# robot-learning-freiburg/MM-DistillNet

Measured on AMD Instinct MI355X. Metric: distillation-step images/sec (3 teachers + audio student, D2, bs=8), higher is better.
Workload: dtype f32; 1 GPU; BASELINE configs[2]: full 3-teacher (RGB+thermal+depth) -> audio student distillation step, EfficientDet-D2, 512x512, per-GPU batch 8, fwd+losses+bwd+all-reduce+Adam; global_batch=8, image_size=512, parallelism=dp1, graph=True, full=False

## Files before the change

### mm_distillnet_amd/csrc/pw_rows.hip

```cpp
#include "common.h"
#include "pw_args.h"
#include <cstdlib>

#define RW_AFF 1
#define RW_SWISH 2
#define RW_GATE 4
#define RW_ABL_NOSTORE 256
#define RW_ABL_NOFETCH 512
#define RW_ABL_NOMFMA 1024

struct RowsArgs {
  int LDB;
  int nslabs;
  int spw;
  int cpp;
  int pcols;
  int npanels, bpp;
  int mode;
  int nlev;
};

typedef float f32x2 __attribute__((ext_vector_type(2)));
typedef __attribute__((address_space(3))) void* lds_vptr;
typedef const __attribute__((address_space(1))) void* glb_vptr;

template <int NKK, int C>
__global__ __launch_bounds__(512, 2) void pw_rows_kernel(PwArgs a, RowsArgs ra) {
  extern __shared__ float smem[];
  const int K = NKK * 8, N = a.N, LDB = ra.LDB, pcols = ra.pcols;
  float* const sB = smem;
  float* const sCoef = sB + pcols * LDB;
  float* const sEp = sCoef + 2 * K;
  float* const sStat = sEp + 3 * pcols;
  const int tid = threadIdx.x, lane = tid & 63, r = lane & 15, g = lane >> 4;
  const int wave = __builtin_amdgcn_readfirstlane(tid >> 6);
  const int panel = blockIdx.x / ra.bpp, bi = blockIdx.x - panel * ra.bpp;
  const int n0p = panel * pcols;

  const int slot = bi * 4 + (wave & 3), nslot = ra.bpp * 4;
  const int q_beg = (int)((long long)slot * ra.nslabs / nslot), q_end = (int)((long long)(slot + 1) * ra.nslabs / nslot);
  const int q_mid = q_beg + (q_end - q_beg + 1) / 2;
  const int s_beg = (wave < 4) ? q_beg : q_mid, s_end = (wave < 4) ? q_mid : q_end;
  f32x2 an[NKK], gn[NKK];
  int lev_n = 0, Mv_n = a.M, srow0_n = 0, rpi_n = a.rows_per_image;
    auto fetch = [&](int s) {
      const int row0 = s * 16;
      lev_n = 0; Mv_n = a.M; srow0_n = 0; rpi_n = a.rows_per_image;
      if (a.pyr.n) {
        lev_n = __builtin_amdgcn_readfirstlane(pyr_level_of_row(a.pyr, row0));
        srow0_n = a.pyr.row0[lev_n]; rpi_n = a.pyr.H[lev_n] * a.pyr.W[lev_n]; Mv_n = srow0_n + a.pyr.B * rpi_n;
      }
      const int row = min(row0 + r, Mv_n - 1);
      const float* xp = a.x + (size_t)row * K + 2 * g;
#pragma unroll
      for (int kk = 0; kk < NKK; ++kk) an[kk] = *reinterpret_cast<const f32x2*>(xp + kk * 8);
      if (ra.mode & RW_GATE) {
        const float* gp = a.gate + (size_t)(row / rpi_n) * K + 2 * g;
#pragma unroll
        for (int kk = 0; kk < NKK; ++kk) gn[kk] = *reinterpret_cast<const f32x2*>(gp + kk * 8);
      }
    };
  if (s_beg < s_end) fetch(s_beg);
  {
    const int f4 = K >> 2, spr = f4 + 1, total = pcols * spr;
    const int nI = (total + 63) >> 6;
    for (int ii = wave; ii < nI; ii += 8) {
      const int slot = ii * 64 + lane;
      const int n = slot / spr, k4 = slot - n * spr;
      const float* src = a.w + (size_t)min(n0p + n, N - 1) * K + min(k4, f4 - 1) * 4;
      if (slot < total && k4 < f4)
        __builtin_amdgcn_global_load_lds((glb_vptr)(uintptr_t)src, (lds_vptr)(uintptr_t)(sB + ii * 256), 16, 0, 0);
    }
    if (ra.mode & RW_AFF)
      for (int k = tid; k < K; k += 512) {
        float sc, sh;
        if (a.in_bn.stats) bn_live_coef(a.in_bn, k, sc, sh);
        else { sc = a.in_scale[k]; sh = a.in_shift[k]; }
        sCoef[k] = sc; sCoef[K + k] = sh;
      }
    for (int c = tid; c < pcols; c += 512) {
      const int col = n0p + c;
      const bool ok = col < N;
      sEp[c] = (a.bias && ok) ? a.bias[col] : 0.f;
      sEp[pcols + c] = (a.out_scale && ok) ? a.out_scale[col] : 1.f;
      sEp[2 * pcols + c] = (a.out_scale && ok) ? a.out_shift[col] : 0.f;
    }
    for (int i = tid; i < ra.nlev * 2 * pcols; i += 512) sStat[i] = 0.f;
  }
  asm volatile("s_waitcnt vmcnt(0)" ::: "memory");
  __syncthreads();

  if (s_beg < s_end) {
    for (int s = s_beg; s < s_end; ++s) {
      const int row0 = s * 16;
      const int lev = lev_n, Mv = Mv_n, srow0 = srow0_n, rpi = rpi_n;
      f32x2 ac[NKK];
#pragma unroll
      for (int kk = 0; kk < NKK; ++kk) ac[kk] = an[kk];
      if (ra.mode & RW_AFF) {
#pragma unroll
        for (int kk = 0; kk < NKK; ++kk) {
          const f32x2 sc = *reinterpret_cast<const f32x2*>(&sCoef[kk * 8 + 2 * g]);
          const f32x2 sh = *reinterpret_cast<const f32x2*>(&sCoef[K + kk * 8 + 2 * g]);
          ac[kk].x = ac[kk].x * sc.x + sh.x; ac[kk].y = ac[kk].y * sc.y + sh.y;
        }
      }
      if (ra.mode & RW_SWISH) {
#pragma unroll
        for (int kk = 0; kk < NKK; ++kk) { ac[kk].x = mmd_swish(ac[kk].x); ac[kk].y = mmd_swish(ac[kk].y); }
      }
      if (ra.mode & RW_GATE) {
#pragma unroll
        for (int kk = 0; kk < NKK; ++kk) { ac[kk].x *= gn[kk].x; ac[kk].y *= gn[kk].y; }
      }
      if (s + 1 < s_end && !(ra.mode & RW_ABL_NOFETCH)) fetch(s + 1);
      const bool rows_full = row0 + 16 <= Mv;
      size_t off[4]; bool rok[4];
#pragma unroll
      for (int i = 0; i < 4; ++i) {
        const int row = row0 + 4 * g + i;
        rok[i] = row < Mv;
        const int rr = rok[i] ? row : row0;
        if (a.y_batch_stride) {
          const int img = (rr - srow0) / rpi;
          const long long yoff = a.pyr.n ? a.yoff_lev[lev] : a.y_offset;
          off[i] = (size_t)img * a.y_batch_stride + yoff + (size_t)(rr - srow0 - img * rpi) * N;
        } else {
          off[i] = (size_t)rr * N;
        }
      }
      for (int ch = 0; ch < ra.cpp; ++ch) {
        const int cbase = ch * C * 16;
        if (n0p + cbase >= N) break;
        const bool full = rows_full && (n0p + cbase + C * 16 <= N);
        const int c0 = n0p + cbase + r;
        float res[C][4];
        if (a.residual) {
#pragma unroll
          for (int j = 0; j < C; ++j)
#pragma unroll
            for (int i = 0; i < 4; ++i) res[j][i] = (c0 + j * 16 < N && rok[i]) ? a.residual[off[i] + c0 + j * 16] : 0.f;
        }
        f32x4 acc[C];
#pragma unroll
        for (int j = 0; j < C; ++j) acc[j] = f32x4{0.f, 0.f, 0.f, 0.f};
        typedef const __attribute__((address_space(3))) f32x2* lds_f2p;
        const unsigned bp0 = (unsigned)(uintptr_t)(lds_vptr)(uintptr_t)(sB + (cbase + r) * LDB + 2 * g);
#pragma unroll
        for (int kk = 0; kk < NKK; ++kk) {
          if ((ra.mode & RW_ABL_NOMFMA) && kk > 0) break;
          f32x2 b[C];
          unsigned bpk = bp0 + kk * 32;
          asm volatile("" : "+v"(bpk));
#pragma unroll
          for (int j = 0; j < C; ++j) b[j] = *(lds_f2p)(uintptr_t)(bpk + j * 16 * LDB * 4);
#pragma unroll
          for (int j = 0; j < C; ++j) acc[j] = __builtin_amdgcn_mfma_f32_16x16x4f32(ac[kk].x, b[j].x, acc[j], 0, 0, 0);
#pragma unroll
          for (int j = 0; j < C; ++j) acc[j] = __builtin_amdgcn_mfma_f32_16x16x4f32(ac[kk].y, b[j].y, acc[j], 0, 0, 0);
        }
        const float* ep = sEp + cbase + r;
        if (a.bias) {
#pragma unroll
          for (int j = 0; j < C; ++j) { const float bias = ep[j * 16]; acc[j] += bias; }
        }
        if (ra.nlev) {
#pragma unroll
          for (int j = 0; j < C; ++j) {
            float ssum = 0.f, ssq = 0.f;
            const bool cok = c0 + j * 16 < N;
#pragma unroll
            for (int i = 0; i < 4; ++i) {
              const float v = (full || (cok && rok[i])) ? acc[j][i] : 0.f;
              ssum += v; ssq += v * v;
            }
            ssum += __shfl_xor(ssum, 16, 64); ssq += __shfl_xor(ssq, 16, 64);
            ssum += __shfl_xor(ssum, 32, 64); ssq += __shfl_xor(ssq, 32, 64);
            if (g == 0 && cok) {
              atomicAdd(&sStat[(lev * 2) * pcols + cbase + j * 16 + r], ssum);
              atomicAdd(&sStat[(lev * 2 + 1) * pcols + cbase + j * 16 + r], ssq);
            }
          }
        }
        if (a.out_scale) {
#pragma unroll
          for (int j = 0; j < C; ++j) { const float osc = ep[pcols + j * 16], osh = ep[2 * pcols + j * 16]; acc[j] = acc[j] * osc + osh; }
        }
        if (a.out_act == MMD_ACT_SWISH) {
#pragma unroll
          for (int j = 0; j < C; ++j)
#pragma unroll
            for (int i = 0; i < 4; ++i) acc[j][i] = mmd_swish(acc[j][i]);
        } else if (a.out_act == MMD_ACT_SIGMOID) {
#pragma unroll
          for (int j = 0; j < C; ++j)
#pragma unroll
            for (int i = 0; i < 4; ++i) acc[j][i] = mmd_sigmoid(acc[j][i]);
        }
        if (a.residual) {
#pragma unroll
          for (int j = 0; j < C; ++j)
#pragma unroll
            for (int i = 0; i < 4; ++i) acc[j][i] += res[j][i];
        }
        if (!(ra.mode & RW_ABL_NOSTORE)) {
          float* yp[4];
#pragma unroll
          for (int i = 0; i < 4; ++i) yp[i] = a.y + off[i] + c0;
          if (full) {
#pragma unroll
            for (int j = 0; j < C; ++j)
#pragma unroll
              for (int i = 0; i < 4; ++i) yp[i][j * 16] = acc[j][i];
          } else {
#pragma unroll
            for (int j = 0; j < C; ++j)
#pragma unroll
              for (int i = 0; i < 4; ++i)
                if (c0 + j * 16 < N && rok[i]) yp[i][j * 16] = acc[j][i];
          }
        }
      }
    }
  }
  if (ra.nlev) {
    __syncthreads();
    double* base = a.stats_ws ? a.stats_ws + (size_t)(blockIdx.x % a.ws_slots) * 2 * N : a.stats;
    for (int i = tid; i < ra.nlev * 2 * pcols; i += 512) {
      const int l = i / (2 * pcols), rem = i - l * 2 * pcols, which = rem / pcols, c = rem - which * pcols;
      const int col = n0p + c;
      const float v = sStat[i];
      if (col < N && v != 0.f) atomicAdd(&base[(a.pyr.n ? 2 * (size_t)l * a.lev_stride : 0) + (size_t)which * N + col], (double)v);
    }
  }
}

typedef void (*RowsKern)(PwArgs, RowsArgs);
template <int C>
static RowsKern rows_pick_k(int nkk) {
  switch (nkk) {
    case 2: return pw_rows_kernel<2, C>;
    case 3: return pw_rows_kernel<3, C>;
    case 4: return pw_rows_kernel<4, C>;
    case 6: return pw_rows_kernel<6, C>;
    case 11: return pw_rows_kernel<11, C>;
    case 12: return pw_rows_kernel<12, C>;
    case 14: return pw_rows_kernel<14, C>;
    case 15: return pw_rows_kernel<15, C>;
    case 16: return pw_rows_kernel<16, C>;
    default: return nullptr;
  }
}
static RowsKern rows_pick(int nkk, int c) {
  return c == 7 ? rows_pick_k<7>(nkk) : c == 4 ? rows_pick_k<4>(nkk) : c == 3 ? rows_pick_k<3>(nkk) : c == 1 ? rows_pick_k<1>(nkk) : nullptr;
}


int pw_rows_try(PwArgs& a, hipStream_t stream) {
  static const int off = getenv("MMD_NO_ROWS") ? 1 : 0;
  static const int lds_blk = getenv("MMD_ROWS_LDS") ? atoi(getenv("MMD_ROWS_LDS")) : 120 * 1024;
  if (off || a.bf16 || a.bb.z || a.xs.z || a.st.Cin) return 0;
  const int M = a.M, K = a.K, N = a.N;
  if (K < 16 || K > 128 || (K & 7)) return 0;
  static const int all = getenv("MMD_ROWS_ALL") ? 1 : 0;
  if (a.form == MMD_PW_FORM_TILED || a.form == MMD_PW_FORM_LONGK || a.form == MMD_PW_FORM_SLAB) return 0;
  if (!all && a.form != MMD_PW_FORM_ROWS && (M < 32768 || a.stats || N < 48)) return 0;
  if (a.in_act != MMD_ACT_NONE && a.in_act != MMD_ACT_SWISH) return 0;
  if (a.gate && (a.pyr.n || (a.rows_per_image & 15))) return 0;
  const int nkk = K / 8;
  const int tiles = cdiv(N, 16);
  const int nslabs = cdiv(M, 16);
  int C = 1; double best = -1.0;
  const int cands[4] = {7, 4, 3, 1};
  for (int ci = 0; ci < 4; ++ci) {
    const int c = cands[ci];
    const double eff = (double)tiles / (cdiv(tiles, c) * c) * (c == 1 ? 0.85 : 1.0);
    if (eff > best + 1e-9) { best = eff; C = c; }
  }
  static const int small_slabs = getenv("MMD_ROWS_SMALL") ? atoi(getenv("MMD_ROWS_SMALL")) : 512;
  if (nslabs * cdiv(tiles, C) < small_slabs && nslabs < small_slabs) C = 1;
  RowsKern kern = rows_pick(nkk, C);
  if (!kern) return 0;
  RowsArgs ra{};
  ra.LDB = K + 4;
  ra.nslabs = nslabs;
  const int nchunks = cdiv(tiles, C);
  const int chunk_bytes = C * 16 * ra.LDB * 4;
  int cpp = lds_blk / chunk_bytes; if (cpp < 1) cpp = 1; if (cpp > nchunks) cpp = nchunks;
  while (cpp > 1 && (long long)nslabs * cdiv(nchunks, cpp) < 1024) --cpp;
  ra.cpp = cpp; ra.pcols = cpp * C * 16; ra.npanels = cdiv(nchunks, cpp);
  ra.mode = ((a.in_scale || a.in_bn.stats) ? RW_AFF : 0) | (a.in_act == MMD_ACT_SWISH ? RW_SWISH : 0) | (a.gate ? RW_GATE : 0);
  static const int abl = (getenv("MMD_DEV") && getenv("MMD_ROWS_ABL")) ? atoi(getenv("MMD_ROWS_ABL")) : 0;
  ra.mode |= abl;
  ra.nlev = a.stats ? (a.pyr.n ? a.pyr.n : 1) : 0;
  const size_t lds = ((size_t)ra.pcols * ra.LDB + 2 * K + 3 * ra.pcols + (size_t)ra.nlev * 2 * ra.pcols) * sizeof(float);
  if (lds > 150 * 1024) return 0;
  static const int blk_target = getenv("MMD_ROWS_BLK") ? atoi(getenv("MMD_ROWS_BLK")) : 256;
  int maxblk = blk_target;
  if (a.stats && !a.stats_ws && maxblk > 128 * ra.npanels) maxblk = 128 * ra.npanels;
  int bpp = maxblk / ra.npanels; if (bpp < 1) bpp = 1;
  if (bpp > cdiv(nslabs, 8)) bpp = cdiv(nslabs, 8);
  ra.spw = cdiv(nslabs, bpp * 4);
  ra.bpp = bpp;
  static bool attr_done[17][8];
  if (!attr_done[nkk][C]) {
    hipFuncSetAttribute((const void*)kern, hipFuncAttributeMaxDynamicSharedMemorySize, 160 * 1024);
    attr_done[nkk][C] = true;
  }
  hipLaunchKernelGGL(kern, dim3(ra.npanels * bpp), dim3(512), lds, stream, a, ra);
  return 1;
}
```

Baseline: 602.7 images/sec.

## Fuse BN-backward prologue and preceding BN/swish grad reductions into rows pointwise kernel

Adds a BB template variant of the rows pointwise kernel that evaluates the batch-norm/activation backward on the input operand in the prologue. It optionally writes dz, accumulates dgamma/dbeta, and fuses per-image reductions for a following swish/BN backward (p5) into the epilogue through LDS and atomics. Previously these backward pointwise GEMMs fell back to other kernel forms, with separate elementwise and reduction passes. The change adds LDS use, atomics and restrictive eligibility conditions, and uses a larger block count for small-LDS cases.

```diff
diff --git a/mm_distillnet_amd/csrc/pw_rows.hip b/mm_distillnet_amd/csrc/pw_rows.hip
--- a/mm_distillnet_amd/csrc/pw_rows.hip
+++ b/mm_distillnet_amd/csrc/pw_rows.hip
@@ -24,14 +24,17 @@
 typedef __attribute__((address_space(3))) void* lds_vptr;
 typedef const __attribute__((address_space(1))) void* glb_vptr;
 
-template <int NKK, int C>
+template <int NKK, int C, int BB = 0>
 __global__ __launch_bounds__(512, 2) void pw_rows_kernel(PwArgs a, RowsArgs ra) {
   extern __shared__ float smem[];
   const int K = NKK * 8, N = a.N, LDB = ra.LDB, pcols = ra.pcols;
+  constexpr int NCO = BB ? 5 : 2;
   float* const sB = smem;
   float* const sCoef = sB + pcols * LDB;
-  float* const sEp = sCoef + 2 * K;
+  float* const sEp = sCoef + NCO * K;
   float* const sStat = sEp + 3 * pcols;
+  float* const sP5c = sStat + ra.nlev * 2 * pcols;
+  float* const sP5 = sP5c + 4 * pcols;
   const int tid = threadIdx.x, lane = tid & 63, r = lane & 15, g = lane >> 4;
   const int wave = __builtin_amdgcn_readfirstlane(tid >> 6);
   const int panel = blockIdx.x / ra.bpp, bi = blockIdx.x - panel * ra.bpp;
@@ -42,6 +45,7 @@
   const int q_mid = q_beg + (q_end - q_beg + 1) / 2;
   const int s_beg = (wave < 4) ? q_beg : q_mid, s_end = (wave < 4) ? q_mid : q_end;
   f32x2 an[NKK], gn[NKK];
+  float rs_n = 1.f;
   int lev_n = 0, Mv_n = a.M, srow0_n = 0, rpi_n = a.rows_per_image;
     auto fetch = [&](int s) {
       const int row0 = s * 16;
@@ -54,7 +58,12 @@
       const float* xp = a.x + (size_t)row * K + 2 * g;
 #pragma unroll
       for (int kk = 0; kk < NKK; ++kk) an[kk] = *reinterpret_cast<const f32x2*>(xp + kk * 8);
-      if (ra.mode & RW_GATE) {
+      if constexpr (BB) {
+        const float* zp = a.bb.z + (size_t)row * K + 2 * g;
+#pragma unroll
+        for (int kk = 0; kk < NKK; ++kk) gn[kk] = *reinterpret_cast<const f32x2*>(zp + kk * 8);
+        rs_n = a.bb.mul_b ? a.bb.mul_b[row / a.bb.rows_per_image] : 1.f;
+      } else if (ra.mode & RW_GATE) {
         const float* gp = a.gate + (size_t)(row / rpi_n) * K + 2 * g;
 #pragma unroll
         for (int kk = 0; kk < NKK; ++kk) gn[kk] = *reinterpret_cast<const f32x2*>(gp + kk * 8);
@@ -71,7 +80,18 @@
       if (slot < total && k4 < f4)
         __builtin_amdgcn_global_load_lds((glb_vptr)(uintptr_t)src, (lds_vptr)(uintptr_t)(sB + ii * 256), 16, 0, 0);
     }
-    if (ra.mode & RW_AFF)
+    if constexpr (BB) {
+      bn_bwd_tab_fill(a.bb, K, sCoef, tid, 512);
+      if (a.bb.dgamma && blockIdx.x == 0)
+        for (int c = tid; c < K; c += 512) { a.bb.dgamma[c] += (float)a.bb.sums[K + c]; a.bb.dbeta[c] += (float)a.bb.sums[c]; }
+      if (a.p5.z) {
+        for (int c = tid; c < pcols; c += 512) {
+          const int col = min(n0p + c, N - 1);
+          sP5c[c] = a.p5.scale[col]; sP5c[pcols + c] = a.p5.shift[col]; sP5c[2 * pcols + c] = a.p5.mean[col]; sP5c[3 * pcols + c] = a.p5.invstd[col];
+        }
+        for (int i = tid; i < 10 * pcols; i += 512) sP5[i] = 0.f;
+      }
+    } else if (ra.mode & RW_AFF)
       for (int k = tid; k < K; k += 512) {
         float sc, sh;
         if (a.in_bn.stats) bn_live_coef(a.in_bn, k, sc, sh);
@@ -90,6 +110,7 @@
   asm volatile("s_waitcnt vmcnt(0)" ::: "memory");
   __syncthreads();
 
+  const int p5_img0 = (BB && a.p5.z) ? (int)((long long)(bi * 4) * ra.nslabs / nslot) * 16 / a.p5.rows_per_image : 0;
   if (s_beg < s_end) {
     for (int s = s_beg; s < s_end; ++s) {
       const int row0 = s * 16;
@@ -97,7 +118,19 @@
       f32x2 ac[NKK];
 #pragma unroll
       for (int kk = 0; kk < NKK; ++kk) ac[kk] = an[kk];
-      if (ra.mode & RW_AFF) {
+      if constexpr (BB) {
+        const bool dz_st = a.bb.dz_out && panel == 0 && row0 + r < Mv;
+        float* const dzp = a.bb.dz_out + (size_t)(row0 + r) * K + 2 * g;
+#pragma unroll
+        for (int kk = 0; kk < NKK; ++kk) {
+          const float* t = &sCoef[kk * 8 + 2 * g];
+          const f32x2 a1 = *reinterpret_cast<const f32x2*>(t), a2 = *reinterpret_cast<const f32x2*>(t + K), a3 = *reinterpret_cast<const f32x2*>(t + 2 * K);
+          const f32x2 mu = *reinterpret_cast<const f32x2*>(t + 3 * K), sh = *reinterpret_cast<const f32x2*>(t + 4 * K);
+          ac[kk].x = bn_bwd_eval(ac[kk].x, gn[kk].x, rs_n, a.bb.act, a1.x, a2.x, a3.x, mu.x, sh.x);
+          ac[kk].y = bn_bwd_eval(ac[kk].y, gn[kk].y, rs_n, a.bb.act, a1.y, a2.y, a3.y, mu.y, sh.y);
+          if (dz_st) *reinterpret_cast<f32x2*>(dzp + kk * 8) = ac[kk];
+        }
+      } else if (ra.mode & RW_AFF) {
 #pragma unroll
         for (int kk = 0; kk < NKK; ++kk) {
           const f32x2 sc = *reinterpret_cast<const f32x2*>(&sCoef[kk * 8 + 2 * g]);
@@ -140,6 +173,15 @@
           for (int j = 0; j < C; ++j)
 #pragma unroll
             for (int i = 0; i < 4; ++i) res[j][i] = (c0 + j * 16 < N && rok[i]) ? a.residual[off[i] + c0 + j * 16] : 0.f;
+        }
+        float pz[BB ? C : 1][4];
+        if constexpr (BB) {
+          if (a.p5.z) {
+#pragma unroll
+            for (int j = 0; j < C; ++j)
+#pragma unroll
+              for (int i = 0; i < 4; ++i) pz[j][i] = a.p5.z[off[i] + min(c0 + j * 16, N - 1)];
+          }
         }
         f32x4 acc[C];
 #pragma unroll
@@ -203,6 +245,32 @@
 #pragma unroll
             for (int i = 0; i < 4; ++i) acc[j][i] += res[j][i];
         }
+        if constexpr (BB) {
+          if (a.p5.z) {
+            float* const dst = sP5 + (row0 / a.p5.rows_per_image - p5_img0) * 5 * pcols + cbase + r;
+#pragma unroll
+            for (int j = 0; j < C; ++j) {
+              const float* q = sP5c + cbase + j * 16 + r;
+              const float sc = q[0], sh = q[pcols], mu = q[2 * pcols], is = q[3 * pcols];
+              const bool cok = c0 + j * 16 < N;
+              float t[5] = {0.f, 0.f, 0.f, 0.f, 0.f};
+#pragma unroll
+              for (int i = 0; i < 4; ++i) {
+                const float zv = pz[j][i], gv = acc[j][i];
+                const float u = zv * sc + sh;
+                const float sg = mmd_sigmoid(u);
+                const float sp = sg * (1.0f + u * (1.0f - sg));
+                const float xh = (zv - mu) * is;
+                if (full || (cok && rok[i])) { t[0] += gv * (u * sg); t[1] += gv * sp; t[2] += gv * sp * xh; t[3] += sp; t[4] += sp * xh; }
+              }
+#pragma unroll
+              for (int k = 0; k < 5; ++k) {
+                t[k] += __shfl_xor(t[k], 16, 64); t[k] += __shfl_xor(t[k], 32, 64);
+                if (g == 0 && cok) atomicAdd(&dst[k * pcols + j * 16], t[k]);
+              }
+            }
+          }
+        }
         if (!(ra.mode & RW_ABL_NOSTORE)) {
           float* yp[4];
 #pragma unroll
@@ -220,6 +288,17 @@
                 if (c0 + j * 16 < N && rok[i]) yp[i][j * 16] = acc[j][i];
           }
         }
+      }
+    }
+  }
+  if constexpr (BB) {
+    if (a.p5.z) {
+      __syncthreads();
+      for (int i = tid; i < 10 * pcols; i += 512) {
+        const int sl = i / (5 * pcols), rem = i - sl * 5 * pcols, k = rem / pcols, c = rem - k * pcols;
+        const int col = n0p + c, img = p5_img0 + sl;
+        const float v = sP5[i];
+        if (col < N && img < a.p5.B && v != 0.f) atomicAdd(&a.p5.out[((size_t)k * a.p5.B + img) * N + col], v);
       }
     }
   }
@@ -251,6 +330,9 @@
     default: return nullptr;
   }
 }
+static RowsKern rows_pick_bb(int nkk) {
+  return nkk == 2 ? pw_rows_kernel<2, 3, 1> : nkk == 3 ? pw_rows_kernel<3, 3, 1> : nkk == 6 ? pw_rows_kernel<6, 3, 1> : nullptr;
+}
 static RowsKern rows_pick(int nkk, int c) {
   return c == 7 ? rows_pick_k<7>(nkk) : c == 4 ? rows_pick_k<4>(nkk) : c == 3 ? rows_pick_k<3>(nkk) : c == 1 ? rows_pick_k<1>(nkk) : nullptr;
 }
@@ -259,12 +341,16 @@
 int pw_rows_try(PwArgs& a, hipStream_t stream) {
   static const int off = getenv("MMD_NO_ROWS") ? 1 : 0;
   static const int lds_blk = getenv("MMD_ROWS_LDS") ? atoi(getenv("MMD_ROWS_LDS")) : 120 * 1024;
-  if (off || a.bf16 || a.bb.z || a.xs.z || a.st.Cin) return 0;
+  if (off || a.bf16 || a.xs.z || a.st.Cin) return 0;
   const int M = a.M, K = a.K, N = a.N;
   if (K < 16 || K > 128 || (K & 7)) return 0;
+  const bool bb = a.bb.z != nullptr;
+  if (bb && ((K != 16 && K != 24 && K != 48) || (N & 15) || a.stats || a.pyr.n || a.y_batch_stride || a.gate || a.in_scale || a.in_bn.stats ||
+             a.in_act != MMD_ACT_NONE || (a.p5.z && (a.p5.rows_per_image & 15)))) return 0;
   static const int all = getenv("MMD_ROWS_ALL") ? 1 : 0;
   if (a.form == MMD_PW_FORM_TILED || a.form == MMD_PW_FORM_LONGK || a.form == MMD_PW_FORM_SLAB) return 0;
   if (!all && a.form != MMD_PW_FORM_ROWS && (M < 32768 || a.stats || N < 48)) return 0;
+  if (bb && !all && a.form != MMD_PW_FORM_ROWS && K == 48) return 0;
   if (a.in_act != MMD_ACT_NONE && a.in_act != MMD_ACT_SWISH) return 0;
   if (a.gate && (a.pyr.n || (a.rows_per_image & 15))) return 0;
   const int nkk = K / 8;
@@ -279,7 +365,8 @@
   }
   static const int small_slabs = getenv("MMD_ROWS_SMALL") ? atoi(getenv("MMD_ROWS_SMALL")) : 512;
   if (nslabs * cdiv(tiles, C) < small_slabs && nslabs < small_slabs) C = 1;
-  RowsKern kern = rows_pick(nkk, C);
+  if (bb) C = 3;
+  RowsKern kern = bb ? rows_pick_bb(nkk) : rows_pick(nkk, C);
   if (!kern) return 0;
   RowsArgs ra{};
   ra.LDB = K + 4;
@@ -293,19 +380,22 @@
   static const int abl = (getenv("MMD_DEV") && getenv("MMD_ROWS_ABL")) ? atoi(getenv("MMD_ROWS_ABL")) : 0;
   ra.mode |= abl;
   ra.nlev = a.stats ? (a.pyr.n ? a.pyr.n : 1) : 0;
-  const size_t lds = ((size_t)ra.pcols * ra.LDB + 2 * K + 3 * ra.pcols + (size_t)ra.nlev * 2 * ra.pcols) * sizeof(float);
+  const size_t lds = ((size_t)ra.pcols * ra.LDB + (bb ? 5 : 2) * K + 3 * ra.pcols + (size_t)ra.nlev * 2 * ra.pcols +
+                      (a.p5.z ? 14 * ra.pcols : 0)) * sizeof(float);
   if (lds > 150 * 1024) return 0;
   static const int blk_target = getenv("MMD_ROWS_BLK") ? atoi(getenv("MMD_ROWS_BLK")) : 256;
-  int maxblk = blk_target;
+  static const int blk_target_bb = getenv("MMD_ROWS_BB_BLK") ? atoi(getenv("MMD_ROWS_BB_BLK")) : 512;
+  int maxblk = bb ? (lds <= 78 * 1024 ? blk_target_bb : 256) : blk_target;
   if (a.stats && !a.stats_ws && maxblk > 128 * ra.npanels) maxblk = 128 * ra.npanels;
   int bpp = maxblk / ra.npanels; if (bpp < 1) bpp = 1;
   if (bpp > cdiv(nslabs, 8)) bpp = cdiv(nslabs, 8);
   ra.spw = cdiv(nslabs, bpp * 4);
   ra.bpp = bpp;
+  if (a.p5.z && cdiv(nslabs, bpp) > a.p5.rows_per_image / 16) return 0;
   static bool attr_done[17][8];
-  if (!attr_done[nkk][C]) {
+  if (!attr_done[nkk][bb ? 0 : C]) {
     hipFuncSetAttribute((const void*)kern, hipFuncAttributeMaxDynamicSharedMemorySize, 160 * 1024);
-    attr_done[nkk][C] = true;
+    attr_done[nkk][bb ? 0 : C] = true;
   }
   hipLaunchKernelGGL(kern, dim3(ra.npanels * bpp), dim3(512), lds, stream, a, ra);
   return 1;
```

After: 602.7 images/sec, median of 3. About the same (+0.0%).
